# ttanida/rgrg

Hardware: AMD Instinct MI355X
Metric: images/sec full 29-region report gen, 512x512 CXR, greedy max_len=128 (higher is better)
Workload: dtype bf16; 1 GPU; full_model.generate() batch=32/GPU, 29 regions, greedy max_len=128, bf16 autocast: 16-bit detector, 16-bit decode GEMMs + K/V cache, hipGraph-captured decode step (BASELINE configs[2]); global_batch=32, parallelism=single GPU, weights=seeded random init (rgrg_amd.synth, profile bench), hipGraph_decode=True

## Files before the change

### include/rgrg_hip.h

```cpp
#ifndef RGRG_HIP_H_
#define RGRG_HIP_H_

#include <stdint.h>

#ifdef __cplusplus
extern "C" {
#endif

#define RGRG_OK 0
#define RGRG_EINVAL (-1)
#define RGRG_EHIP (-2)
#define RGRG_ESTATE (-3)

#define RGRG_ACT_NONE 0
#define RGRG_ACT_RELU 1
#define RGRG_ACT_GELU_NEW 2

const char* rgrg_last_error(void);
int rgrg_abi_version(void);
int rgrg_device_arch(int dev, char* buf, int buflen);

int rgrg_linear_f32(const float* A, const float* W, const float* scale, const float* shift, const float* R,
                    float* Y, int M, int N, int K, int ldy, int act, int splitk, float* ws, void* stream);
int rgrg_conv2d_nhwc_f32(const float* X, const float* W, const float* scale, const float* shift, const float* R,
// ... 93 lines not shown
int rgrg_bf16_to_f32(const uint16_t* src, float* dst, int64_t n, int fp16, void* stream);
int rgrg_conv2d_nhwc_bf16(const uint16_t* X16, const uint16_t* Wb, const float* shift, const uint16_t* R16, float* Y,
                          uint16_t* Y16, int B, int H, int Wd, int Cin, int Cout, int KH, int KW, int stride, int pad,
                          int act, int fp16, void* stream);
int rgrg_linear_bf16w_f32(const float* A, const uint16_t* Wb, const float* shift, const float* R, float* Y, int M,
                          int N, int K, int ldy, int act, int fp16, void* stream);
int rgrg_linear_bf16_f32(const uint16_t* A16, const uint16_t* Wb, const float* shift, const float* R, float* Y,
                         uint16_t* Y16, int M, int N, int K, int ldy, int act, int fp16, void* stream);
int rgrg_debug_linear_bf16_tile(const uint16_t* A16, const uint16_t* Wb, const float* shift, const float* R, float* Y,
                                int M, int N, int K, int ldy, int act, int tile, int lda, int ldw, int fp16, void* stream);
int rgrg_debug_linear_bf16_train(const uint16_t* A16, const uint16_t* Wb, const float* shift, const float* R, float* Y,
                                 uint16_t* Y16, uint16_t* Ypre16, const uint16_t* G16, int M, int N, int K, int ldy, int act,
                                 int tile, int fp16, void* stream);
int rgrg_debug_linear_bf16_argmax(const uint16_t* A16, const uint16_t* Wb, const float* shift, int M, int N, int K,
                                  float* cand_val, int* cand_idx, int fp16, void* stream);
int rgrg_debug_ln_fold16(const float* w, const float* gain, const float* beta, const float* bias, uint16_t* wb, float* colsum,
                         float* shift, int N, int K, int fp16, void* stream);
int rgrg_debug_linear_bf16_ln(const uint16_t* A16, const uint16_t* Wb, const float* shift, const float* R, float* Y,
                              uint16_t* Yb16, float* stats_out, const float* ln_stats, const float* ln_colsum, int M, int N,
                              int K, int ldy, int act, int fp16, void* stream);
int rgrg_debug_linear_bf16_ln_kv(const uint16_t* A16, const uint16_t* Wb, const float* shift, float* Y, const float* ln_stats,
                                 const float* ln_colsum, uint16_t* kcache, uint16_t* vcache, const int* step_dev, int M, int H,
                                 int T_slots, int K, int ldy, int fp16, void* stream);
int rgrg_debug_linear_bf16_ln_kp(const uint16_t* A16, const uint16_t* Wb, const float* shift, const float* R, float* Y,
                                 uint16_t* Y16, uint16_t* Yb16, float* stats_out, const float* ln_stats, const float* ln_colsum,
                                 int M, int N, int K, int ldy, int act, int fp16, int kp, void* stream);
int rgrg_debug_attn_decode(const float* qkv, int ld_qkv, void* kcache, void* vcache, const int* step_dev, float* out,
                           uint16_t* out16, int S, int H, int T_slots, const int* src, const float* kmask, int kv16, int fp16,
                           int ni, int frag_out, int max_workgroups, void* stream);
int rgrg_debug_attn_decode_qonly(const float* q, int ld_q, const void* kcache, const void* vcache, const int* step_dev, float* out,
// ... 45 lines not shown
```

### rgrg_amd/_hip.py

```python
from __future__ import annotations

import ctypes as C
import os
from typing import Optional

from . import build as _build

c_float_p = C.c_void_p
_i, _f, _p = C.c_int, C.c_float, C.c_void_p

ACT_NONE, ACT_RELU, ACT_GELU_NEW = 0, 1, 2
ABI_VERSION = 25


class RgrgHipError(RuntimeError):
    pass


class DecoderLayerWeights(C.Structure):
    _fields_ = [(n, _p) for n in ("ln1_g", "ln1_b", "ln2_g", "ln2_b", "c_attn_w", "c_attn_b", "attn_proj_w",
                                  "attn_proj_b", "c_fc_w", "c_fc_b", "mlp_proj_w", "mlp_proj_b")]


class DecoderWeights(C.Structure):
    _fields_ = [("n_layer", _i), ("d_model", _i), ("n_head", _i), ("vocab", _i), ("wte", _p), ("lnf_g", _p),
                ("lnf_b", _p), ("fst0_w", _p), ("fst0_b", _p), ("fst2_w", _p), ("fst2_b", _p), ("ukv_w", _p),
                ("ukv_b", _p), ("layers", C.POINTER(DecoderLayerWeights))]
# ... 35 lines not shown
    "rgrg_decoder_cache_plane": (_i, [_p, _i, _i, C.POINTER(C.c_void_p), C.POINTER(_i), C.POINTER(_i), C.POINTER(_i)]),
    "rgrg_transpose_pad_f32": (_i, [_p, _p, _i, _i, _i, _p]),
    "rgrg_colsum_f32": (_i, [_p, _p, _i, _i, _p]),
    "rgrg_relu_backward_f32": (_i, [_p, _p, C.c_int64, _p]),
    "rgrg_bce_with_logits_masked_backward_f32": (_i, [_p, _p, _p, C.c_float, _i, C.c_float, _p, _i, _p]),
    "rgrg_adamw_step_f32": (_i, [_p, _p, _p, _p, C.c_int64, C.c_float, C.c_float, C.c_float, C.c_float, C.c_float, _i, C.c_float, _p]),
    "rgrg_adamw_multi_step_f32": (_i, [_p, _i, C.c_float, C.c_float, C.c_float, C.c_float, C.c_float, _i, C.c_float, _p]),
    "rgrg_f32_to_bf16": (_i, [_p, _p, C.c_int64, _i, _p]),
    "rgrg_bf16_to_f32": (_i, [_p, _p, C.c_int64, _i, _p]),
    "rgrg_conv2d_nhwc_bf16": (_i, [_p, _p, _p, _p, _p, _p, _i, _i, _i, _i, _i, _i, _i, _i, _i, _i, _i, _p]),
    "rgrg_linear_bf16w_f32": (_i, [_p, _p, _p, _p, _p, _i, _i, _i, _i, _i, _i, _p]),
    "rgrg_linear_bf16_f32": (_i, [_p, _p, _p, _p, _p, _p, _i, _i, _i, _i, _i, _i, _p]),
    "rgrg_debug_linear_bf16_tile": (_i, [_p, _p, _p, _p, _p, _i, _i, _i, _i, _i, _i, _i, _i, _i, _p]),
    "rgrg_debug_linear_bf16_train": (_i, [_p, _p, _p, _p, _p, _p, _p, _p, _i, _i, _i, _i, _i, _i, _i, _p]),
    "rgrg_debug_linear_bf16_argmax": (_i, [_p, _p, _p, _i, _i, _i, _p, _p, _i, _p]),
    "rgrg_debug_ln_fold16": (_i, [_p, _p, _p, _p, _p, _p, _p, _i, _i, _i, _p]),
    "rgrg_debug_linear_bf16_ln": (_i, [_p, _p, _p, _p, _p, _p, _p, _p, _p, _i, _i, _i, _i, _i, _i, _p]),
    "rgrg_debug_linear_bf16_ln_kp": (_i, [_p, _p, _p, _p, _p, _p, _p, _p, _p, _p, _i, _i, _i, _i, _i, _i, _i, _p]),
    "rgrg_debug_attn_decode": (_i, [_p, _i, _p, _p, _p, _p, _p, _i, _i, _i, _p, _p, _i, _i, _i, _i, _i, _p]),
    "rgrg_debug_linear_bf16_ln_kv": (_i, [_p, _p, _p, _p, _p, _p, _p, _p, _p, _i, _i, _i, _i, _i, _i, _p]),
    "rgrg_debug_attn_decode_qonly": (_i, [_p, _i, _p, _p, _p, _p, _p, _i, _i, _i, _i, _i, _p]),
    "rgrg_debug_attn_decode_kv8": (_i, [_p, _i, _p, _p, _p, _p, _p, _i, _i, _i, _p, _p, _i, _i, _p]),
    "rgrg_debug_attn_prefill": (_i, [_p, _p, _i, _i, _p, _p, _p, _p, _i, _i, _i, _i, C.c_uint64, C.c_uint32, _f, _i, _p]),
    "rgrg_debug_attn_backward_f32": (_i, [_p, _p, _i, _i, _p, _p, _p, _p, _p, _p, _p, _p, _i, _i, _i, C.c_uint64, C.c_uint32, _f,
                                          _i, _f, _p]),
    "rgrg_debug_attn_train16": (_i, [_i, _p, _p, _i, _i, _p, _p, _p, _p, _p, _p, _i, _i, _i, C.c_uint64, C.c_uint32, _f, _f, _i, _p]),
    "rgrg_decoder_copy_last_logits": (_i, [_p, _p, _i, _p]),
    "rgrg_box_match_f32": (_i, [_p, _p, _i, _p, C.c_int64, _p, _i, _i, _f, _f, _i, _p, _p, _p]),
    "rgrg_balanced_sample": (_i, [_p, _p, _i, _p, _p, C.c_uint64, _i, _i, _i, _i, _i, _p, _p, _p, _p, _p]),
    "rgrg_rpn_loss_sampled_f32": (_i, [_p, _i, _i, _p, _p, _i, _p, _p, _p, _p, _i, _i, _i, _p, _p]),
# ... 67 lines not shown
```

### rgrg_amd/csrc/gemm_bf16.hip

```cpp
#include "internal.h"

namespace rgrg {

typedef short bf16x8 __attribute__((ext_vector_type(8)));
typedef short bf16x4 __attribute__((ext_vector_type(4)));
typedef unsigned short u16;

struct GemmBf16Params {
    const float* A;
    const u16* A16;
    const u16* Wb;
    const float* shift;
    const float* R;
    float* Y;
    u16* Y16;
    int M, N, K, ldy, act;
    int lda = 0, ldw = 0;
    int cH = 0, cW = 0, cCin = 0, cKH = 0, cKW = 0, cStride = 1, cPad = 0, cOH = 0, cOW = 0;
    const u16* R16 = nullptr;
    int f16 = 0;
    u16* Yb16 = nullptr;
    float* stats_out = nullptr;
    const float* ln_stats = nullptr;
    const float* ln_colsum = nullptr;
// ... 603 lines not shown
    }
}

template <int TAG>
__device__ __forceinline__ void pp_dma4(const u16* base, unsigned char* dst, const int (&v)[4], int soff) {
    const __amdgpu_buffer_rsrc_t r = bf16_rsrc(base);
#pragma unroll
    for (int j = 0; j < 4; ++j) __builtin_amdgcn_raw_ptr_buffer_load_lds(r, (lds_ptr_t)(dst + j * 8192), 16, v[j], soff, 0, 0);
}
template <int TAG>
__device__ __forceinline__ void pp_dma2(const u16* base, unsigned char* dst, int v0, int v1, int soff) {
    const __amdgpu_buffer_rsrc_t r = bf16_rsrc(base);
    __builtin_amdgcn_raw_ptr_buffer_load_lds(r, (lds_ptr_t)dst, 16, v0, soff, 0, 0);
    __builtin_amdgcn_raw_ptr_buffer_load_lds(r, (lds_ptr_t)(dst + 1024), 16, v1, soff, 0, 0);
}
template <bool F16>
__global__ __launch_bounds__(512) void gemm_bf16_pp_kernel(const GemmBf16Params p, const int mtiles, const int ntiles) {
    constexpr int BM = 256, BN = 256, BK = 64, MI = 4, NI = 2;
    constexpr int STAGE = (BM + BN) * 128, WOFF = BM * 128;
    constexpr int TAG = F16 ? 901 : 900;
    extern __shared__ __attribute__((aligned(16))) unsigned char pp_smem[];
    const int tid = threadIdx.x, lane = tid & 63;
    const int wave = __builtin_amdgcn_readfirstlane(tid >> 6);
    const int g = wave >> 2, wq = wave & 3;
    int t = blockIdx.x;
    {
        const int total = mtiles * ntiles, q = total >> 3, r = total & 7, x = t & 7, i = t >> 3;
        t = (x < r ? x * (q + 1) : r * (q + 1) + (x - r) * q) + i;
    }
    int tn, tm;
    if (p.gm <= 0 || p.gm >= mtiles) {
        tn = t / mtiles; tm = t - tn * mtiles;
    } else {
        const int gsz = p.gm * ntiles, gi = t / gsz, r = t - gi * gsz;
        const int rows = min(p.gm, mtiles - gi * p.gm);
        tn = r / rows; tm = gi * p.gm + (r - tn * rows);
    }
    const int m0 = tm * BM, n0 = tn * BN;
    const int nk = p.K / BK;
    const int lda = p.lda ? p.lda : p.K, ldw = p.ldw ? p.ldw : p.K;
    const u16* abase = p.A16 + (size_t)m0 * lda;
    const u16* wbase = p.Wb + (size_t)n0 * ldw;
    const int lrow = lane >> 3, lch = lane & 7;
    auto src_off = [&](int row0, int limit, int ld) { const int row = row0 + lrow; return min(row, limit) * ld * 2 + ((lch ^ ((row >> 1) & 7)) << 4); };
    const int ra0 = (g == 0 ? 192 : 0) + wq * 16, ra1 = (g == 0 ? 128 : 64) + wq * 16;
    const int rw0 = (g == 0 ? 0 : 128) + wq * 16, rw1 = rw0 + 64;
    const int va00 = src_off(ra0, p.M - 1 - m0, lda), va01 = src_off(ra0 + 8, p.M - 1 - m0, lda);
    const int va10 = src_off(ra1, p.M - 1 - m0, lda), va11 = src_off(ra1 + 8, p.M - 1 - m0, lda);
    const int vw00 = src_off(rw0, p.N - 1 - n0, ldw), vw01 = src_off(rw0 + 8, p.N - 1 - n0, ldw);
    const int vw10 = src_off(rw1, p.N - 1 - n0, ldw), vw11 = src_off(rw1 + 8, p.N - 1 - n0, ldw);
    unsigned char* const da0 = pp_smem + ra0 * 128;
    unsigned char* const da1 = pp_smem + ra1 * 128;
    unsigned char* const dw0 = pp_smem + WOFF + rw0 * 128;
    unsigned char* const dw1 = pp_smem + WOFF + rw1 * 128;
    const int frow = lane & 31, fh = lane >> 5, fsw = (frow >> 1) & 7;
    int foff[4];
#pragma unroll
    for (int ks = 0; ks < 4; ++ks) foff[ks] = frow * 128 + (((2 * ks + fh) ^ fsw) << 4);
    const unsigned char* const fa_base = pp_smem + g * (128 * 128);
    const unsigned char* const fb_base = pp_smem + WOFF + wq * (64 * 128);

    f32x16 acc[MI][NI];
#pragma unroll
    for (int mi = 0; mi < MI; ++mi)
#pragma unroll
        for (int ni = 0; ni < NI; ++ni)
#pragma unroll
            for (int r = 0; r < 16; ++r) acc[mi][ni][r] = 0.f;
    bf16x8 fa[4][2], fb[4][NI];
    float esh[NI];
#pragma unroll
    for (int ni = 0; ni < NI; ++ni) esh[ni] = p.shift ? p.shift[min(n0 + wq * 64 + ni * 32 + (lane & 31), p.N - 1)] : 0.f;
    const int dbg = __builtin_amdgcn_readfirstlane(p.dbg);
    if (dbg) {
#pragma unroll
        for (int ks = 0; ks < 4; ++ks)
#pragma unroll
            for (int i = 0; i < 2; ++i) { fa[ks][i] = bf16x8{1, 2, 3, 4, 5, 6, 7, 8}; fb[ks][i] = bf16x8{8, 7, 6, 5, 4, 3, 2, 1}; }
    }

#define PP_READ_A(ST_, H_)                                                                                       \
    if (!(dbg & 1)) {                                                                                            \
        const unsigned char* sa_ = fa_base + (ST_) * STAGE + (H_) * (64 * 128);                                  \
        _Pragma("unroll") for (int ks = 0; ks < 4; ++ks)                                                         \
            _Pragma("unroll") for (int m2 = 0; m2 < 2; ++m2)                                                     \
                fa[ks][m2] = *reinterpret_cast<const bf16x8*>(sa_ + m2 * 4096 + foff[ks]);                       \
    }
#define PP_READ_W(ST_)                                                                                           \
    if (!(dbg & 1)) {                                                                                            \
        const unsigned char* sw_ = fb_base + (ST_) * STAGE;                                                      \
        _Pragma("unroll") for (int ks = 0; ks < 4; ++ks)                                                         \
            _Pragma("unroll") for (int ni = 0; ni < NI; ++ni)                                                    \
                fb[ks][ni] = *reinterpret_cast<const bf16x8*>(sw_ + ni * 4096 + foff[ks]);                       \
    }
// ... 14 lines not shown
    }
#define PP_END_READ(FIRST_, DO_, TA_, WAIT_)                                                                                  \
    {                                                                                                                          \
        if ((DO_) && !(dbg & 2)) {                                                                                             \
            pp_dma2<TAG>(abase, ((FIRST_) ? da0 : da1) + ((TA_) & 1) * STAGE, (FIRST_) ? va00 : va10, (FIRST_) ? va01 : va11, (TA_) * (BK * 2)); \
            if (!(FIRST_)) {                                                                                                   \
                pp_dma2<TAG>(wbase, dw0 + ((TA_) & 1) * STAGE, vw00, vw01, (TA_) * (BK * 2));                                  \
                pp_dma2<TAG>(wbase, dw1 + ((TA_) & 1) * STAGE, vw10, vw11, (TA_) * (BK * 2));                                  \
            }                                                                                                                  \
        }                                                                                                                      \
        asm volatile("s_waitcnt lgkmcnt(0)" ::: "memory");                                                                     \
        if (dbg & 2) wait_vmcnt<0>(); else wait_vmcnt<WAIT_>();                                                                \
        PP_BAR()                                                                                                               \
    }

    {
        int vpa[4], vpw[4];
#pragma unroll
        for (int j = 0; j < 4; ++j) {
            vpa[j] = src_off((j * 8 + wave) * 8, p.M - 1 - m0, lda);
            vpw[j] = src_off((j * 8 + wave) * 8, p.N - 1 - n0, ldw);
        }
        unsigned char* const dst = pp_smem + wave * 1024;
        pp_dma4<TAG>(wbase, dst + WOFF, vpw, 0);
        pp_dma4<TAG>(abase, dst, vpa, 0);
        pp_dma4<TAG>(wbase, dst + STAGE + WOFF, vpw, BK * 2);
        pp_dma4<TAG>(abase, dst + STAGE, vpa, BK * 2);
    }
    wait_vmcnt<8>();
    PP_BAR()

#define PP_TILE_G0(D0_, W0_, D2_, W2_)                                              \
    {                                                                               \
        const int cur = kt & 1;                                                     \
        PP_READ_A(cur, 0) PP_READ_W(cur)                                            \
        PP_END_READ(true, D0_, kt + 1, W0_)                                         \
        PP_MUL(0)                                                                   \
        PP_BAR()                                                                    \
        PP_READ_A(cur, 1)                                                           \
        PP_END_READ(false, D2_, kt + 2, W2_)                                        \
        PP_MUL(1)                                                                   \
        PP_BAR()                                                                    \
    }
#define PP_TILE_G1(FIRSTKT_, D1_, W1_, D3_, W3_)                                    \
// ... 20 lines not shown
        PP_TILE_G1(true, 1, 2, 1, 8)
        for (kt = 1; kt < nk - 2; ++kt) PP_TILE_G1(false, 1, 8, 1, 8)
        PP_TILE_G1(false, 0, 6, 0, 0)
        ++kt;
        PP_TILE_G1(false, 0, 0, 0, 0)
        PP_MUL(1)
    }
#undef PP_TILE_G0
#undef PP_TILE_G1
#undef PP_END_READ
#undef PP_MUL
#undef PP_READ_A
#undef PP_READ_W
#undef PP_BAR

    if (dbg & 8) {
        float z = 0.f;
#pragma unroll
        for (int mi = 0; mi < MI; ++mi)
#pragma unroll
            for (int ni = 0; ni < NI; ++ni)
#pragma unroll
                for (int r = 0; r < 16; ++r) z += acc[mi][ni][r];
        if (z == 12345.678f) p.Y[0] = z;
        return;
    }
    if (p.cand_val) {
        __syncthreads();
        float* cv = reinterpret_cast<float*>(pp_smem);
        int* ci = reinterpret_cast<int*>(pp_smem + 4096);
        const int ccol = lane & 31;
#pragma unroll
        for (int mi = 0; mi < MI; ++mi) {
            float bv[16];
            int bi[16];
            const int c0 = n0 + wq * 64 + ccol, c1 = c0 + 32;
#pragma unroll
            for (int r = 0; r < 16; ++r) {
                const float v0 = c0 < p.N ? acc[mi][0][r] + esh[0] : -INFINITY;
                const float v1 = c1 < p.N ? acc[mi][1][r] + esh[1] : -INFINITY;
                const bool hi = v1 > v0;
                bv[r] = hi ? v1 : v0;
                bi[r] = hi ? c1 : c0;
            }
#define PP_CAND_STEP(CNT_, XOR_)                                                                   \
    {                                                                                              \
        const bool up = (lane & (XOR_)) != 0;                                                      \
        _Pragma("unroll") for (int j = 0; j < (CNT_); ++j) {                                       \
            const float keep_v = up ? bv[j + (CNT_)] : bv[j], send_v = up ? bv[j] : bv[j + (CNT_)]; \
            const int keep_i = up ? bi[j + (CNT_)] : bi[j], send_i = up ? bi[j] : bi[j + (CNT_)];   \
            const float ov = __shfl_xor(send_v, (XOR_), 64);                                       \
            const int oi = __shfl_xor(send_i, (XOR_), 64);                                         \
            const bool take = ov > keep_v || (ov == keep_v && oi < keep_i);                        \
            bv[j] = take ? ov : keep_v;                                                            \
            bi[j] = take ? oi : keep_i;                                                            \
        }                                                                                          \
    }
            PP_CAND_STEP(8, 16) PP_CAND_STEP(4, 8) PP_CAND_STEP(2, 4) PP_CAND_STEP(1, 2)
#undef PP_CAND_STEP
            {
                const float ov = __shfl_xor(bv[0], 1, 64);
                const int oi = __shfl_xor(bi[0], 1, 64);
                if (ov > bv[0] || (ov == bv[0] && oi < bi[0])) { bv[0] = ov; bi[0] = oi; }
            }
            if ((lane & 1) == 0) {
                const int r = ((lane >> 4) & 1) * 8 + ((lane >> 3) & 1) * 4 + ((lane >> 2) & 1) * 2 + ((lane >> 1) & 1);
                const int lrow_t = mi * 32 + (r & 3) + 8 * (r >> 2) + 4 * (lane >> 5);
                cv[(g * 4 + wq) * 128 + lrow_t] = bv[0];
                ci[(g * 4 + wq) * 128 + lrow_t] = bi[0];
            }
        }
        __syncthreads();
        if (tid < 256) {
            const int gg = tid >> 7, lr = tid & 127, row = m0 + tid;
            float best = cv[(gg * 4) * 128 + lr];
            int idx = ci[(gg * 4) * 128 + lr];
#pragma unroll
            for (int q = 1; q < 4; ++q) {
                const float v = cv[(gg * 4 + q) * 128 + lr];
                if (v > best) { best = v; idx = ci[(gg * 4 + q) * 128 + lr]; }
            }
            if (row < p.M) {
                p.cand_val[(size_t)row * ntiles + tn] = best;
                p.cand_idx[(size_t)row * ntiles + tn] = idx;
            }
        }
        return;
    }
    const int ccol = lane & 31, crow4 = 4 * (lane >> 5);
#pragma unroll
    for (int mi = 0; mi < MI; ++mi)
#pragma unroll
        for (int ni = 0; ni < NI; ++ni) {
            const int col = n0 + wq * 64 + ni * 32 + ccol;
            const int colc = min(col, p.N - 1);
            const int rbase = m0 + g * 128 + mi * 32 + crow4;
            const float sh = esh[ni];
            float rv[16], vv[16];
#pragma unroll
            for (int r = 0; r < 16; ++r) rv[r] = 0.f;
            if (p.R) {
#pragma unroll
                for (int r = 0; r < 16; ++r) {
                    const int row = min(rbase + (r & 3) + 8 * (r >> 2), p.M - 1);
                    rv[r] = p.R[(size_t)row * p.ldy + colc];
                }
            }
            if (p.G16) {
#pragma unroll
                for (int r = 0; r < 16; ++r) {
                    const int row = min(rbase + (r & 3) + 8 * (r >> 2), p.M - 1);
                    rv[r] = from16<F16>(p.G16[(size_t)row * p.ldy + colc]);
// ... 13 lines not shown
                for (int r = 0; r < 16; ++r) vv[r] = apply_act_fast(acc[mi][ni][r] + sh + rv[r], p.act);
            }
            if (col < p.N) {
#pragma unroll
                for (int r = 0; r < 16; ++r) {
                    const int dr = (r & 3) + 8 * (r >> 2);
                    if (rbase + dr < p.M) {
                        const size_t o = (size_t)rbase * p.ldy + col + (size_t)(dr * p.ldy);
                        if (p.Y16) p.Y16[o] = (u16)to16<F16>(vv[r]);
                        else if (p.N > 8192) __builtin_nontemporal_store(vv[r], &p.Y[o]);
                        else p.Y[o] = vv[r];
                    }
                }
            }
        }
}

__global__ __launch_bounds__(256) void f32_to_bf16_kernel(const float* __restrict__ src, u16* __restrict__ dst, size_t n, int f16) {
    for (size_t i = (size_t)blockIdx.x * blockDim.x + threadIdx.x; i < n; i += (size_t)gridDim.x * blockDim.x)
        dst[i] = (u16)to16_rt(src[i], f16);
}

template <int BM, int BN, int THREADS>
static int launch_bf16_cfg(const GemmBf16Params& p, hipStream_t st) {
    constexpr size_t lds = (size_t)(2 * BM + 2 * BN) * LDB * sizeof(u16);
    const int mtiles = (p.M + BM - 1) / BM, ntiles = (p.N + BN - 1) / BN;
#define RGRG_W_LAUNCH(A16_, F16_) hipLaunchKernelGGL((gemm_bf16w_kernel<BM, BN, THREADS, A16_, F16_>), dim3(mtiles * ntiles), dim3(THREADS), lds, st, p, mtiles, ntiles)
    if (p.A16) { if (p.f16) RGRG_W_LAUNCH(true, true); else RGRG_W_LAUNCH(true, false); }
    else { if (p.f16) RGRG_W_LAUNCH(false, true); else RGRG_W_LAUNCH(false, false); }
#undef RGRG_W_LAUNCH
// ... 23 lines not shown
    RGRG_G_ATTR(false, false, 3); RGRG_G_ATTR(false, true, 3);
#undef RGRG_G_ATTR
    return RGRG_OK;
}
template <int BM, int BN>
static int glds_attrs() {
    int rc;
    if ((rc = glds_attr<BM, BN, 2>()) || (rc = glds_attr<BM, BN, 3>())) return rc;
    return glds_attr<BM, BN, 4>();
}

static int gemm_gm_override();
#include "gemm_kp.inc"

constexpr int PP_LDS = 2 * (256 + 256) * 128;

int init_gemm_bf16_attrs() {
    static bool done = false;
    if (done) return RGRG_OK;
    int rc;
    if ((rc = bf16_attr<128, 128, 512>()) || (rc = bf16_attr<64, 64, 256>())) return rc;
    if ((rc = glds_attrs<128, 128>()) || (rc = glds_attrs<64, 64>()) || (rc = glds_attrs<128, 64>()) || (rc = glds_attrs<64, 128>())) return rc;
    RGRG_HIP(hipFuncSetAttribute(reinterpret_cast<const void*>(&gemm_bf16_pp_kernel<false>), hipFuncAttributeMaxDynamicSharedMemorySize, PP_LDS));
    RGRG_HIP(hipFuncSetAttribute(reinterpret_cast<const void*>(&gemm_bf16_pp_kernel<true>), hipFuncAttributeMaxDynamicSharedMemorySize, PP_LDS));
    if ((rc = kp_attr<128, 128, 2>()) || (rc = kp_attr<64, 64, 4>()) || (rc = kp_attr<64, 64, 3>()) || (rc = kp_attr<128, 64, 3>()) || (rc = kp_attr<64, 128, 3>()) || (rc = kp_attr<64, 64, 2>()) || (rc = pr_attrs())) return rc;
    done = true;
    return RGRG_OK;
}

static int gemm_gm_override() {
    static const int v = [] { const char* e = getenv("RGRG_GEMM_GM"); return e ? atoi(e) : 0; }();
    return v;
}

template <int BM, int BN, int NST>
static int launch_glds_cfg(const GemmBf16Params& p0, hipStream_t st) {
    GemmBf16Params p = p0;
    const int mtiles = (p.M + BM - 1) / BM, ntiles = (p.N + BN - 1) / BN;
    if (p.gm == 0) {
// ... 10 lines not shown
    else { if (p.f16) RGRG_G_LAUNCH(false, true, 0); else RGRG_G_LAUNCH(false, false, 0); }
#undef RGRG_G_LAUNCH
    RGRG_LAUNCH_CHECK();
    return RGRG_OK;
}
template <int BM, int BN>
static int launch_glds_nst(const GemmBf16Params& p, int nst, hipStream_t st) {
    if (nst == 2) return launch_glds_cfg<BM, BN, 2>(p, st);
    if (nst == 3) return launch_glds_cfg<BM, BN, 3>(p, st);
    return launch_glds_cfg<BM, BN, 4>(p, st);
}

static bool pp_eligible(const GemmBf16Params& p) {
    return !p.cCin && !p.Yb16 && !p.ln_colsum && !p.R16 && p.K >= 256 && p.K % 64 == 0;
}
static int launch_pp(const GemmBf16Params& p0, hipStream_t st) {
    GemmBf16Params p = p0;
    const int mtiles = (p.M + 255) / 256, ntiles = (p.N + 255) / 256;
    if (p.gm == 0) {
        const int o = gemm_gm_override();
        p.gm = o < 0 ? 0 : o > 0 ? o : (mtiles > 8 ? 8 : 0);
    }
    { const char* e = getenv("RGRG_PP_DBG"); p.dbg = e ? atoi(e) : 0; }
    if (p.f16) hipLaunchKernelGGL(gemm_bf16_pp_kernel<true>, dim3(mtiles * ntiles), dim3(512), PP_LDS, st, p, mtiles, ntiles);
    else hipLaunchKernelGGL(gemm_bf16_pp_kernel<false>, dim3(mtiles * ntiles), dim3(512), PP_LDS, st, p, mtiles, ntiles);
    RGRG_LAUNCH_CHECK();
    return RGRG_OK;
}
static bool pp_enabled() {
    static const bool v = [] { const char* e = getenv("RGRG_GEMM_PP"); return !e || atoi(e) != 0; }();
    return v;
}

static bool pp_lm_head() {
    static const bool v = [] { const char* e = getenv("RGRG_GEMM_PP_LMHEAD"); return !e || atoi(e) != 0; }();
    return v;
}

static int launch_glds(const GemmBf16Params& p, int tile, hipStream_t st) {
    int shape = tile & 15, nst = tile >> 4;
    if (p.kv_k && shape >= 5) { set_error("bf16 GEMM: only the LDS-DMA kernel has the K/V-cache epilogue (tile %d)", tile); return RGRG_EINVAL; }
    switch (shape) {
        case 6: return launch_kp_cfg<128, 128, 2>(p, st);
        case 7: return launch_kp_cfg<64, 64, 4>(p, st);
        case 8: return launch_kp_cfg<128, 64, 3>(p, st);
        case 9: return launch_kp_cfg<64, 128, 3>(p, st);
        case 10: return launch_kp_cfg<64, 64, 3>(p, st);
        case 11: return launch_kp_auto(p, st);
        case 12: return launch_pr(p, st);
        case 13: return launch_kp_cfg<64, 64, 2>(p, st);
    }
    if (shape == 5) {
        if (!pp_eligible(p)) { set_error("bf16 GEMM: the 256 x 256 kernel does not take this variant"); return RGRG_EINVAL; }
        return launch_pp(p, st);
    }
    if (shape == 0 && pp_enabled() && pp_eligible(p)) {
        const long tiles_pp = (long)((p.M + 255) / 256) * ((p.N + 255) / 256);
        if (p.M >= 2048 && tiles_pp >= 192) return launch_pp(p, st);
        if (p.M >= 512 && p.N >= 32768 && tiles_pp >= 512 && pp_lm_head()) return launch_pp(p, st);
    }
    if (shape == 0 && p.ln_colsum && p.M <= 320) {
        static const int o = [] { const char* e = getenv("RGRG_CONS_TILE_SMALLM"); return e ? atoi(e) : 0; }();
        if (o) { shape = o & 15; nst = o >> 4; }
    }
    if (shape == 0) {
        const long tiles_big = (long)((p.M + 127) / 128) * ((p.N + 127) / 128);
        if (p.N <= 64) { shape = 3; nst = 2; }
        else if (tiles_big >= 512) { shape = 1; nst = 2; }
        else if (p.K >= 8192 && tiles_big >= 192) { shape = 1; nst = 2; }
// ... 130 lines not shown
    p.f16 = fp16 ? 1 : 0;
    p.Ypre16 = Ypre16; p.G16 = G16;
    return launch_glds(p, tile, as_stream(stream));
}

extern "C" int rgrg_debug_linear_bf16_argmax(const uint16_t* A16, const uint16_t* Wb, const float* shift, int M, int N, int K,
                                             float* cand_val, int* cand_idx, int fp16, void* stream) {
    int rc = init_gemm_bf16_attrs();
    if (rc) return rc;
    RGRG_CHECK_ARG(A16 && Wb && cand_val && cand_idx && M > 0 && N > 0 && K >= 256 && K % 256 == 0);
    GemmLnFold f{};
    f.cand_val = cand_val; f.cand_idx = cand_idx;
    return launch_gemm_bf16w_ex(nullptr, A16, Wb, shift, nullptr, nullptr, nullptr, M, N, K, N, RGRG_ACT_NONE, as_stream(stream), fp16, &f);
}

extern "C" int rgrg_debug_linear_bf16_ln(const uint16_t* A16, const uint16_t* Wb, const float* shift, const float* R, float* Y,
                                         uint16_t* Yb16, float* stats_out, const float* ln_stats, const float* ln_colsum, int M,
                                         int N, int K, int ldy, int act, int fp16, void* stream) {
    int rc = init_gemm_bf16_attrs();
    if (rc) return rc;
    RGRG_CHECK_ARG(A16 && Wb && Y);
    GemmLnFold f{};
    f.Yb16 = Yb16; f.stats_out = stats_out; f.ln_stats = ln_stats; f.ln_colsum = ln_colsum;
    return launch_gemm_bf16w_ex(nullptr, A16, Wb, shift, R, Y, nullptr, M, N, K, ldy, act, as_stream(stream), fp16, &f);
}

extern "C" int rgrg_debug_linear_bf16_ln_kv(const uint16_t* A16, const uint16_t* Wb, const float* shift, float* Y, const float* ln_stats,
                                            const float* ln_colsum, uint16_t* kcache, uint16_t* vcache, const int* step_dev, int M, int H,
                                            int T_slots, int K, int ldy, int fp16, void* stream) {
    int rc = init_gemm_bf16_attrs();
// ... 38 lines not shown
```

### rgrg_amd/csrc/runtime.hip

```cpp
#include <stdarg.h>
#include <string.h>

#include "common.h"

namespace rgrg {
static thread_local char g_err[512] = "";
void set_error(const char* fmt, ...) {
    va_list ap;
    va_start(ap, fmt);
    vsnprintf(g_err, sizeof(g_err), fmt, ap);
    va_end(ap);
}
}

extern "C" const char* rgrg_last_error(void) { return rgrg::g_err; }
extern "C" int rgrg_abi_version(void) { return 25; }
extern "C" int rgrg_device_arch(int dev, char* buf, int buflen) {
    RGRG_CHECK_ARG(buf && buflen > 1);
    hipDeviceProp_t prop;
    RGRG_HIP(hipGetDeviceProperties(&prop, dev));
    strncpy(buf, prop.gcnArchName, buflen - 1);
    buf[buflen - 1] = 0;
    return RGRG_OK;
}

#include <chrono>
namespace rgrg {
__global__ void chain_kernel(int* p, int n) {
    if (threadIdx.x == 0 && blockIdx.x == 0) p[0] += n;
}
}
// ... 37 lines not shown
```

Baseline: 89.44 images/sec.

## Make LM-head argmax GEMM persistent, prefetching next tile during epilogue

Adds a WALK variant of the 256x256 ping-pong bf16 GEMM used for the fused LM-head argmax. It launches one workgroup per CU, and each workgroup loops over tiles. Before running the argmax epilogue of the current tile, it issues the DMA prologue for the next tile, so epilogue and tile-launch costs overlap with loads. The variant is on by default when the tile count exceeds the CU count. It uses extra LDS scratch for the epilogue and gives up the per-tile launch parallelism and the grouped raster order beyond the first wave.

```diff
diff --git a/include/rgrg_hip.h b/include/rgrg_hip.h
--- a/include/rgrg_hip.h
+++ b/include/rgrg_hip.h
@@ -131,6 +131,8 @@
                                  int tile, int fp16, void* stream);
 int rgrg_debug_linear_bf16_argmax(const uint16_t* A16, const uint16_t* Wb, const float* shift, int M, int N, int K,
                                   float* cand_val, int* cand_idx, int fp16, void* stream);
+int rgrg_debug_linear_bf16_argmax_walk(const uint16_t* A16, const uint16_t* Wb, const float* shift, int M, int N, int K,
+                                       float* cand_val, int* cand_idx, int fp16, int grid, void* stream);
 int rgrg_debug_ln_fold16(const float* w, const float* gain, const float* beta, const float* bias, uint16_t* wb, float* colsum,
                          float* shift, int N, int K, int fp16, void* stream);
 int rgrg_debug_linear_bf16_ln(const uint16_t* A16, const uint16_t* Wb, const float* shift, const float* R, float* Y,
diff --git a/rgrg_amd/_hip.py b/rgrg_amd/_hip.py
--- a/rgrg_amd/_hip.py
+++ b/rgrg_amd/_hip.py
@@ -10,7 +10,7 @@
 _i, _f, _p = C.c_int, C.c_float, C.c_void_p
 
 ACT_NONE, ACT_RELU, ACT_GELU_NEW = 0, 1, 2
-ABI_VERSION = 25
+ABI_VERSION = 26
 
 
 class RgrgHipError(RuntimeError):
@@ -76,6 +76,7 @@
     "rgrg_debug_linear_bf16_tile": (_i, [_p, _p, _p, _p, _p, _i, _i, _i, _i, _i, _i, _i, _i, _i, _p]),
     "rgrg_debug_linear_bf16_train": (_i, [_p, _p, _p, _p, _p, _p, _p, _p, _i, _i, _i, _i, _i, _i, _i, _p]),
     "rgrg_debug_linear_bf16_argmax": (_i, [_p, _p, _p, _i, _i, _i, _p, _p, _i, _p]),
+    "rgrg_debug_linear_bf16_argmax_walk": (_i, [_p, _p, _p, _i, _i, _i, _p, _p, _i, _i, _p]),
     "rgrg_debug_ln_fold16": (_i, [_p, _p, _p, _p, _p, _p, _p, _i, _i, _i, _p]),
     "rgrg_debug_linear_bf16_ln": (_i, [_p, _p, _p, _p, _p, _p, _p, _p, _p, _i, _i, _i, _i, _i, _i, _p]),
     "rgrg_debug_linear_bf16_ln_kp": (_i, [_p, _p, _p, _p, _p, _p, _p, _p, _p, _p, _i, _i, _i, _i, _i, _i, _i, _p]),
diff --git a/rgrg_amd/csrc/gemm_bf16.hip b/rgrg_amd/csrc/gemm_bf16.hip
--- a/rgrg_amd/csrc/gemm_bf16.hip
+++ b/rgrg_amd/csrc/gemm_bf16.hip
@@ -641,7 +641,7 @@
     __builtin_amdgcn_raw_ptr_buffer_load_lds(r, (lds_ptr_t)dst, 16, v0, soff, 0, 0);
     __builtin_amdgcn_raw_ptr_buffer_load_lds(r, (lds_ptr_t)(dst + 1024), 16, v1, soff, 0, 0);
 }
-template <bool F16>
+template <bool F16, bool WALK>
 __global__ __launch_bounds__(512) void gemm_bf16_pp_kernel(const GemmBf16Params p, const int mtiles, const int ntiles) {
     constexpr int BM = 256, BN = 256, BK = 64, MI = 4, NI = 2;
     constexpr int STAGE = (BM + BN) * 128, WOFF = BM * 128;
@@ -650,32 +650,55 @@
     const int tid = threadIdx.x, lane = tid & 63;
     const int wave = __builtin_amdgcn_readfirstlane(tid >> 6);
     const int g = wave >> 2, wq = wave & 3;
-    int t = blockIdx.x;
-    {
-        const int total = mtiles * ntiles, q = total >> 3, r = total & 7, x = t & 7, i = t >> 3;
-        t = (x < r ? x * (q + 1) : r * (q + 1) + (x - r) * q) + i;
-    }
-    int tn, tm;
-    if (p.gm <= 0 || p.gm >= mtiles) {
-        tn = t / mtiles; tm = t - tn * mtiles;
-    } else {
-        const int gsz = p.gm * ntiles, gi = t / gsz, r = t - gi * gsz;
-        const int rows = min(p.gm, mtiles - gi * p.gm);
-        tn = r / rows; tm = gi * p.gm + (r - tn * rows);
-    }
-    const int m0 = tm * BM, n0 = tn * BN;
+    const int total = mtiles * ntiles;
     const int nk = p.K / BK;
     const int lda = p.lda ? p.lda : p.K, ldw = p.ldw ? p.ldw : p.K;
-    const u16* abase = p.A16 + (size_t)m0 * lda;
-    const u16* wbase = p.Wb + (size_t)n0 * ldw;
-    const int lrow = lane >> 3, lch = lane & 7;
-    auto src_off = [&](int row0, int limit, int ld) { const int row = row0 + lrow; return min(row, limit) * ld * 2 + ((lch ^ ((row >> 1) & 7)) << 4); };
     const int ra0 = (g == 0 ? 192 : 0) + wq * 16, ra1 = (g == 0 ? 128 : 64) + wq * 16;
     const int rw0 = (g == 0 ? 0 : 128) + wq * 16, rw1 = rw0 + 64;
-    const int va00 = src_off(ra0, p.M - 1 - m0, lda), va01 = src_off(ra0 + 8, p.M - 1 - m0, lda);
-    const int va10 = src_off(ra1, p.M - 1 - m0, lda), va11 = src_off(ra1 + 8, p.M - 1 - m0, lda);
-    const int vw00 = src_off(rw0, p.N - 1 - n0, ldw), vw01 = src_off(rw0 + 8, p.N - 1 - n0, ldw);
-    const int vw10 = src_off(rw1, p.N - 1 - n0, ldw), vw11 = src_off(rw1 + 8, p.N - 1 - n0, ldw);
+    int tn, m0, n0;
+    const u16 *abase, *wbase;
+    int va00, va01, va10, va11, vw00, vw01, vw10, vw11;
+    int vpa[4], vpw[4];
+    float esh[NI];
+    auto set_tile = [&](int pos) {
+        int lrow = lane >> 3, lch = lane & 7;
+        if constexpr (WALK) asm volatile("" : "+v"(lrow), "+v"(lch));
+        int t;
+        {
+            const int q = total >> 3, r = total & 7, x = pos & 7, i = pos >> 3;
+            t = (x < r ? x * (q + 1) : r * (q + 1) + (x - r) * q) + i;
+        }
+        int tm;
+        if (p.gm <= 0 || p.gm >= mtiles) {
+            tn = t / mtiles; tm = t - tn * mtiles;
+        } else {
+            const int gsz = p.gm * ntiles, gi = t / gsz, r = t - gi * gsz;
+            const int rows = min(p.gm, mtiles - gi * p.gm);
+            tn = r / rows; tm = gi * p.gm + (r - tn * rows);
+        }
+        m0 = tm * BM; n0 = tn * BN;
+        abase = p.A16 + (size_t)m0 * lda;
+        wbase = p.Wb + (size_t)n0 * ldw;
+        auto src_off = [&](int row0, int limit, int ld) { const int row = row0 + lrow; return min(row, limit) * ld * 2 + ((lch ^ ((row >> 1) & 7)) << 4); };
+        va00 = src_off(ra0, p.M - 1 - m0, lda); va01 = src_off(ra0 + 8, p.M - 1 - m0, lda);
+        va10 = src_off(ra1, p.M - 1 - m0, lda); va11 = src_off(ra1 + 8, p.M - 1 - m0, lda);
+        vw00 = src_off(rw0, p.N - 1 - n0, ldw); vw01 = src_off(rw0 + 8, p.N - 1 - n0, ldw);
+        vw10 = src_off(rw1, p.N - 1 - n0, ldw); vw11 = src_off(rw1 + 8, p.N - 1 - n0, ldw);
+#pragma unroll
+        for (int j = 0; j < 4; ++j) {
+            vpa[j] = src_off((j * 8 + wave) * 8, p.M - 1 - m0, lda);
+            vpw[j] = src_off((j * 8 + wave) * 8, p.N - 1 - n0, ldw);
+        }
+#pragma unroll
+        for (int ni = 0; ni < NI; ++ni) esh[ni] = p.shift ? p.shift[min(n0 + wq * 64 + ni * 32 + (lane & 31), p.N - 1)] : 0.f;
+    };
+    auto issue_prologue = [&]() {
+        unsigned char* const dst = pp_smem + wave * 1024;
+        pp_dma4<TAG>(wbase, dst + WOFF, vpw, 0);
+        pp_dma4<TAG>(abase, dst, vpa, 0);
+        pp_dma4<TAG>(wbase, dst + STAGE + WOFF, vpw, BK * 2);
+        pp_dma4<TAG>(abase, dst + STAGE, vpa, BK * 2);
+    };
     unsigned char* const da0 = pp_smem + ra0 * 128;
     unsigned char* const da1 = pp_smem + ra1 * 128;
     unsigned char* const dw0 = pp_smem + WOFF + rw0 * 128;
@@ -687,24 +710,10 @@
     const unsigned char* const fa_base = pp_smem + g * (128 * 128);
     const unsigned char* const fb_base = pp_smem + WOFF + wq * (64 * 128);
 
-    f32x16 acc[MI][NI];
-#pragma unroll
-    for (int mi = 0; mi < MI; ++mi)
-#pragma unroll
-        for (int ni = 0; ni < NI; ++ni)
-#pragma unroll
-            for (int r = 0; r < 16; ++r) acc[mi][ni][r] = 0.f;
-    bf16x8 fa[4][2], fb[4][NI];
-    float esh[NI];
-#pragma unroll
-    for (int ni = 0; ni < NI; ++ni) esh[ni] = p.shift ? p.shift[min(n0 + wq * 64 + ni * 32 + (lane & 31), p.N - 1)] : 0.f;
-    const int dbg = __builtin_amdgcn_readfirstlane(p.dbg);
-    if (dbg) {
-#pragma unroll
-        for (int ks = 0; ks < 4; ++ks)
-#pragma unroll
-            for (int i = 0; i < 2; ++i) { fa[ks][i] = bf16x8{1, 2, 3, 4, 5, 6, 7, 8}; fb[ks][i] = bf16x8{8, 7, 6, 5, 4, 3, 2, 1}; }
-    }
+    int pos = blockIdx.x;
+    set_tile(pos);
+    issue_prologue();
+    const int dbg = WALK ? 0 : __builtin_amdgcn_readfirstlane(p.dbg);
 
 #define PP_READ_A(ST_, H_)                                                                                       \
     if (!(dbg & 1)) {                                                                                            \
@@ -749,20 +758,22 @@
         PP_BAR()                                                                                                               \
     }
 
-    {
-        int vpa[4], vpw[4];
-#pragma unroll
-        for (int j = 0; j < 4; ++j) {
-            vpa[j] = src_off((j * 8 + wave) * 8, p.M - 1 - m0, lda);
-            vpw[j] = src_off((j * 8 + wave) * 8, p.N - 1 - n0, ldw);
-        }
-        unsigned char* const dst = pp_smem + wave * 1024;
-        pp_dma4<TAG>(wbase, dst + WOFF, vpw, 0);
-        pp_dma4<TAG>(abase, dst, vpa, 0);
-        pp_dma4<TAG>(wbase, dst + STAGE + WOFF, vpw, BK * 2);
-        pp_dma4<TAG>(abase, dst + STAGE, vpa, BK * 2);
-    }
-    wait_vmcnt<8>();
+    for (;;) {
+    f32x16 acc[MI][NI];
+    bf16x8 fa[4][2], fb[4][NI];
+    if (dbg) {
+#pragma unroll
+        for (int ks = 0; ks < 4; ++ks)
+#pragma unroll
+            for (int i = 0; i < 2; ++i) { fa[ks][i] = bf16x8{1, 2, 3, 4, 5, 6, 7, 8}; fb[ks][i] = bf16x8{8, 7, 6, 5, 4, 3, 2, 1}; }
+    }
+#pragma unroll
+    for (int mi = 0; mi < MI; ++mi)
+#pragma unroll
+        for (int ni = 0; ni < NI; ++ni)
+#pragma unroll
+            for (int r = 0; r < 16; ++r) acc[mi][ni][r] = 0.f;
+    if (!WALK || pos == (int)blockIdx.x) wait_vmcnt<8>(); else wait_vmcnt<0>();
     PP_BAR()
 
 #define PP_TILE_G0(D0_, W0_, D2_, W2_)                                              \
@@ -813,6 +824,18 @@
 #undef PP_READ_W
 #undef PP_BAR
 
+    const int e_tn = tn, e_m0 = m0, e_n0 = n0;
+    const float e_sh[NI] = {esh[0], esh[1]};
+    bool more = false;
+    if constexpr (WALK) {
+        more = pos + (int)gridDim.x < total;
+        if (more) {
+            pos += gridDim.x;
+            set_tile(pos);
+            issue_prologue();
+        }
+    }
+
     if (dbg & 8) {
         float z = 0.f;
 #pragma unroll
@@ -821,30 +844,34 @@
             for (int ni = 0; ni < NI; ++ni)
 #pragma unroll
                 for (int r = 0; r < 16; ++r) z += acc[mi][ni][r];
-        if (z == 12345.678f) p.Y[0] = z;
-        return;
-    }
-    if (p.cand_val) {
-        __syncthreads();
-        float* cv = reinterpret_cast<float*>(pp_smem);
-        int* ci = reinterpret_cast<int*>(pp_smem + 4096);
-        const int ccol = lane & 31;
+        if (z == 12345.678f) *(p.cand_val ? p.cand_val : p.Y) = z;
+        if (!more) break;
+        continue;
+    }
+    if (WALK || p.cand_val) {
+        int lane_e = lane, tid_e = tid;
+        if constexpr (WALK) asm volatile("" : "+v"(lane_e), "+v"(tid_e));
+        if constexpr (!WALK) __syncthreads();
+        unsigned char* const scratch = pp_smem + (WALK ? 2 * STAGE : 0);
+        float* cv = reinterpret_cast<float*>(scratch);
+        int* ci = reinterpret_cast<int*>(scratch + 4096);
+        const int ccol = lane_e & 31;
 #pragma unroll
         for (int mi = 0; mi < MI; ++mi) {
             float bv[16];
             int bi[16];
-            const int c0 = n0 + wq * 64 + ccol, c1 = c0 + 32;
+            const int c0 = e_n0 + wq * 64 + ccol, c1 = c0 + 32;
 #pragma unroll
             for (int r = 0; r < 16; ++r) {
-                const float v0 = c0 < p.N ? acc[mi][0][r] + esh[0] : -INFINITY;
-                const float v1 = c1 < p.N ? acc[mi][1][r] + esh[1] : -INFINITY;
+                const float v0 = c0 < p.N ? acc[mi][0][r] + e_sh[0] : -INFINITY;
+                const float v1 = c1 < p.N ? acc[mi][1][r] + e_sh[1] : -INFINITY;
                 const bool hi = v1 > v0;
                 bv[r] = hi ? v1 : v0;
                 bi[r] = hi ? c1 : c0;
             }
 #define PP_CAND_STEP(CNT_, XOR_)                                                                   \
     {                                                                                              \
-        const bool up = (lane & (XOR_)) != 0;                                                      \
+        const bool up = (lane_e & (XOR_)) != 0;                                                      \
         _Pragma("unroll") for (int j = 0; j < (CNT_); ++j) {                                       \
             const float keep_v = up ? bv[j + (CNT_)] : bv[j], send_v = up ? bv[j] : bv[j + (CNT_)]; \
             const int keep_i = up ? bi[j + (CNT_)] : bi[j], send_i = up ? bi[j] : bi[j + (CNT_)];   \
@@ -862,16 +889,16 @@
                 const int oi = __shfl_xor(bi[0], 1, 64);
                 if (ov > bv[0] || (ov == bv[0] && oi < bi[0])) { bv[0] = ov; bi[0] = oi; }
             }
-            if ((lane & 1) == 0) {
-                const int r = ((lane >> 4) & 1) * 8 + ((lane >> 3) & 1) * 4 + ((lane >> 2) & 1) * 2 + ((lane >> 1) & 1);
-                const int lrow_t = mi * 32 + (r & 3) + 8 * (r >> 2) + 4 * (lane >> 5);
+            if ((lane_e & 1) == 0) {
+                const int r = ((lane_e >> 4) & 1) * 8 + ((lane_e >> 3) & 1) * 4 + ((lane_e >> 2) & 1) * 2 + ((lane_e >> 1) & 1);
+                const int lrow_t = mi * 32 + (r & 3) + 8 * (r >> 2) + 4 * (lane_e >> 5);
                 cv[(g * 4 + wq) * 128 + lrow_t] = bv[0];
                 ci[(g * 4 + wq) * 128 + lrow_t] = bi[0];
             }
         }
         __syncthreads();
-        if (tid < 256) {
-            const int gg = tid >> 7, lr = tid & 127, row = m0 + tid;
+        if (tid_e < 256) {
+            const int gg = tid_e >> 7, lr = tid_e & 127, row = e_m0 + tid_e;
             float best = cv[(gg * 4) * 128 + lr];
             int idx = ci[(gg * 4) * 128 + lr];
 #pragma unroll
@@ -880,21 +907,23 @@
                 if (v > best) { best = v; idx = ci[(gg * 4 + q) * 128 + lr]; }
             }
             if (row < p.M) {
-                p.cand_val[(size_t)row * ntiles + tn] = best;
-                p.cand_idx[(size_t)row * ntiles + tn] = idx;
-            }
-        }
-        return;
-    }
+                p.cand_val[(size_t)row * ntiles + e_tn] = best;
+                p.cand_idx[(size_t)row * ntiles + e_tn] = idx;
+            }
+        }
+        if (!more) break;
+        continue;
+    }
+    if constexpr (!WALK) {
     const int ccol = lane & 31, crow4 = 4 * (lane >> 5);
 #pragma unroll
     for (int mi = 0; mi < MI; ++mi)
 #pragma unroll
         for (int ni = 0; ni < NI; ++ni) {
-            const int col = n0 + wq * 64 + ni * 32 + ccol;
+            const int col = e_n0 + wq * 64 + ni * 32 + ccol;
             const int colc = min(col, p.N - 1);
-            const int rbase = m0 + g * 128 + mi * 32 + crow4;
-            const float sh = esh[ni];
+            const int rbase = e_m0 + g * 128 + mi * 32 + crow4;
+            const float sh = e_sh[ni];
             float rv[16], vv[16];
 #pragma unroll
             for (int r = 0; r < 16; ++r) rv[r] = 0.f;
@@ -938,6 +967,9 @@
                 }
             }
         }
+    }
+    break;
+    }
 }
 
 __global__ __launch_bounds__(256) void f32_to_bf16_kernel(const float* __restrict__ src, u16* __restrict__ dst, size_t n, int f16) {
@@ -991,6 +1023,8 @@
 #include "gemm_kp.inc"
 
 constexpr int PP_LDS = 2 * (256 + 256) * 128;
+constexpr int PP_WALK_LDS = PP_LDS + 8192;
+static int pp_cu_count = 0;
 
 int init_gemm_bf16_attrs() {
     static bool done = false;
@@ -998,8 +1032,15 @@
     int rc;
     if ((rc = bf16_attr<128, 128, 512>()) || (rc = bf16_attr<64, 64, 256>())) return rc;
     if ((rc = glds_attrs<128, 128>()) || (rc = glds_attrs<64, 64>()) || (rc = glds_attrs<128, 64>()) || (rc = glds_attrs<64, 128>())) return rc;
-    RGRG_HIP(hipFuncSetAttribute(reinterpret_cast<const void*>(&gemm_bf16_pp_kernel<false>), hipFuncAttributeMaxDynamicSharedMemorySize, PP_LDS));
-    RGRG_HIP(hipFuncSetAttribute(reinterpret_cast<const void*>(&gemm_bf16_pp_kernel<true>), hipFuncAttributeMaxDynamicSharedMemorySize, PP_LDS));
+    RGRG_HIP(hipFuncSetAttribute(reinterpret_cast<const void*>(&gemm_bf16_pp_kernel<false, false>), hipFuncAttributeMaxDynamicSharedMemorySize, PP_LDS));
+    RGRG_HIP(hipFuncSetAttribute(reinterpret_cast<const void*>(&gemm_bf16_pp_kernel<true, false>), hipFuncAttributeMaxDynamicSharedMemorySize, PP_LDS));
+    RGRG_HIP(hipFuncSetAttribute(reinterpret_cast<const void*>(&gemm_bf16_pp_kernel<false, true>), hipFuncAttributeMaxDynamicSharedMemorySize, PP_WALK_LDS));
+    RGRG_HIP(hipFuncSetAttribute(reinterpret_cast<const void*>(&gemm_bf16_pp_kernel<true, true>), hipFuncAttributeMaxDynamicSharedMemorySize, PP_WALK_LDS));
+    {
+        int dev = 0;
+        RGRG_HIP(hipGetDevice(&dev));
+        RGRG_HIP(hipDeviceGetAttribute(&pp_cu_count, hipDeviceAttributeMultiprocessorCount, dev));
+    }
     if ((rc = kp_attr<128, 128, 2>()) || (rc = kp_attr<64, 64, 4>()) || (rc = kp_attr<64, 64, 3>()) || (rc = kp_attr<128, 64, 3>()) || (rc = kp_attr<64, 128, 3>()) || (rc = kp_attr<64, 64, 2>()) || (rc = pr_attrs())) return rc;
     done = true;
     return RGRG_OK;
@@ -1040,16 +1081,28 @@
 static bool pp_eligible(const GemmBf16Params& p) {
     return !p.cCin && !p.Yb16 && !p.ln_colsum && !p.R16 && p.K >= 256 && p.K % 64 == 0;
 }
-static int launch_pp(const GemmBf16Params& p0, hipStream_t st) {
+static bool pp_walk_enabled() {
+    const char* e = getenv("RGRG_LMHEAD_WALK");
+    return !e || atoi(e) != 0;
+}
+static int launch_pp(const GemmBf16Params& p0, hipStream_t st, int walk_grid = -1) {
     GemmBf16Params p = p0;
     const int mtiles = (p.M + 255) / 256, ntiles = (p.N + 255) / 256;
+    if (walk_grid == 0) walk_grid = (pp_walk_enabled() && pp_cu_count > 0 && mtiles * ntiles > pp_cu_count) ? pp_cu_count : -1;
+    if (walk_grid > 0 && p.cand_val) {
+        if (walk_grid > mtiles * ntiles) walk_grid = mtiles * ntiles;
+        if (p.f16) hipLaunchKernelGGL((gemm_bf16_pp_kernel<true, true>), dim3(walk_grid), dim3(512), PP_WALK_LDS, st, p, mtiles, ntiles);
+        else hipLaunchKernelGGL((gemm_bf16_pp_kernel<false, true>), dim3(walk_grid), dim3(512), PP_WALK_LDS, st, p, mtiles, ntiles);
+        RGRG_LAUNCH_CHECK();
+        return RGRG_OK;
+    }
     if (p.gm == 0) {
         const int o = gemm_gm_override();
         p.gm = o < 0 ? 0 : o > 0 ? o : (mtiles > 8 ? 8 : 0);
     }
     { const char* e = getenv("RGRG_PP_DBG"); p.dbg = e ? atoi(e) : 0; }
-    if (p.f16) hipLaunchKernelGGL(gemm_bf16_pp_kernel<true>, dim3(mtiles * ntiles), dim3(512), PP_LDS, st, p, mtiles, ntiles);
-    else hipLaunchKernelGGL(gemm_bf16_pp_kernel<false>, dim3(mtiles * ntiles), dim3(512), PP_LDS, st, p, mtiles, ntiles);
+    if (p.f16) hipLaunchKernelGGL((gemm_bf16_pp_kernel<true, false>), dim3(mtiles * ntiles), dim3(512), PP_LDS, st, p, mtiles, ntiles);
+    else hipLaunchKernelGGL((gemm_bf16_pp_kernel<false, false>), dim3(mtiles * ntiles), dim3(512), PP_LDS, st, p, mtiles, ntiles);
     RGRG_LAUNCH_CHECK();
     return RGRG_OK;
 }
@@ -1078,7 +1131,7 @@
     }
     if (shape == 5) {
         if (!pp_eligible(p)) { set_error("bf16 GEMM: the 256 x 256 kernel does not take this variant"); return RGRG_EINVAL; }
-        return launch_pp(p, st);
+        return launch_pp(p, st, p.cand_val ? 0 : -1);
     }
     if (shape == 0 && pp_enabled() && pp_eligible(p)) {
         const long tiles_pp = (long)((p.M + 255) / 256) * ((p.N + 255) / 256);
@@ -1239,6 +1292,17 @@
     return launch_gemm_bf16w_ex(nullptr, A16, Wb, shift, nullptr, nullptr, nullptr, M, N, K, N, RGRG_ACT_NONE, as_stream(stream), fp16, &f);
 }
 
+extern "C" int rgrg_debug_linear_bf16_argmax_walk(const uint16_t* A16, const uint16_t* Wb, const float* shift, int M, int N, int K,
+                                                  float* cand_val, int* cand_idx, int fp16, int grid, void* stream) {
+    int rc = init_gemm_bf16_attrs();
+    if (rc) return rc;
+    RGRG_CHECK_ARG(A16 && Wb && cand_val && cand_idx && M > 0 && N > 0 && K >= 256 && K % 256 == 0);
+    GemmBf16Params p{nullptr, A16, Wb, shift, nullptr, nullptr, nullptr, M, N, K, N, RGRG_ACT_NONE};
+    p.f16 = fp16 ? 1 : 0;
+    p.cand_val = cand_val; p.cand_idx = cand_idx;
+    return launch_pp(p, as_stream(stream), grid);
+}
+
 extern "C" int rgrg_debug_linear_bf16_ln(const uint16_t* A16, const uint16_t* Wb, const float* shift, const float* R, float* Y,
                                          uint16_t* Yb16, float* stats_out, const float* ln_stats, const float* ln_colsum, int M,
                                          int N, int K, int ldy, int act, int fp16, void* stream) {
diff --git a/rgrg_amd/csrc/runtime.hip b/rgrg_amd/csrc/runtime.hip
--- a/rgrg_amd/csrc/runtime.hip
+++ b/rgrg_amd/csrc/runtime.hip
@@ -14,7 +14,7 @@
 }
 
 extern "C" const char* rgrg_last_error(void) { return rgrg::g_err; }
-extern "C" int rgrg_abi_version(void) { return 25; }
+extern "C" int rgrg_abi_version(void) { return 26; }
 extern "C" int rgrg_device_arch(int dev, char* buf, int buflen) {
     RGRG_CHECK_ARG(buf && buflen > 1);
     hipDeviceProp_t prop;
```

Result: no change. 89.46 images/sec, median of 3 (+0.0%).
